# Janmajayamall/tfhe-research

Measured on AMD Instinct MI355X. Metric: programmable_bootstraps_per_sec, higher is better.
Workload: dtype f64

## Files before the change

include/tfhe_hip.h:

```cpp
#ifndef TFHE_HIP_H
#define TFHE_HIP_H

#include <stddef.h>
#include <stdint.h>

#ifdef __cplusplus
extern "C" {
#endif

#define TFHE_OK 0
#define TFHE_ERR_INVALID_PARAMS 1
#define TFHE_ERR_UNSUPPORTED 2
#define TFHE_ERR_NO_KEY 3
#define TFHE_ERR_HIP 4
#define TFHE_ERR_INVALID_ARGUMENT 5
#define TFHE_ERR_NO_DEVICE 6
#define TFHE_ERR_EXACTNESS 7
#define TFHE_ERR_IO 8

typedef struct tfhe_decomposer_params {
    uint32_t log_base;
    uint32_t levels;
    uint32_t log_q;
} tfhe_decomposer_params;
// ... 223 lines not shown
                                    uint32_t *bsk_bmmp, uint32_t *ksk, int load);
int tfhe_bootstrapping_key_gen_bmmp_device(tfhe_context *ctx, const uint32_t *lwe_sk,
                                           const uint32_t *glwe_sk, uint32_t *bsk_bmmp, uint32_t *ksk,
                                           int load);

int tfhe_context_set_bootstrap_order(tfhe_context *ctx, int ks_first);

#define TFHE_SHAPE_AUTO 0
#define TFHE_SHAPE_WIDE 1
#define TFHE_SHAPE_TEAM 2
int tfhe_context_set_kernel_shape(tfhe_context *ctx, int shape);

#define TFHE_KS_PATH_AUTO 0
#define TFHE_KS_PATH_SCALAR 1
#define TFHE_KS_PATH_MATRIX 2
int tfhe_context_set_key_switch_path(tfhe_context *ctx, int path);
int tfhe_debug_key_switch_plan(tfhe_context *ctx, size_t batch, int *path, unsigned *grid_x, unsigned *grid_y,
                               unsigned *splits);

int tfhe_context_set_decomposer_alignment(tfhe_context *ctx, int aligned);

#define TFHE_FILE_BSK 1
#define TFHE_FILE_KSK 2
#define TFHE_FILE_LWE 3
#define TFHE_FILE_GLWE 4
#define TFHE_FILE_GGSW 5
#define TFHE_FILE_WORDS 6
#define TFHE_FILE_PKSK 7
#define TFHE_FILE_FLAG_ALIGNED 1u
int tfhe_file_write(const char *path, uint32_t kind, const tfhe_params *params, uint32_t flags,
                    const uint32_t *dims, uint32_t ndims, const uint32_t *data);
// ... 56 lines not shown
```

rust/src/lib.rs:

```rust
use ndarray::{Array1, Array2, Array3};
use std::os::raw::{c_char, c_int, c_void};

#[repr(C)]
#[derive(Clone, Copy)]
pub struct CDecomposerParams { pub log_base: u32, pub levels: u32, pub log_q: u32 }

#[repr(C)]
#[derive(Clone, Copy)]
pub struct CTfheParams {
    pub glwe_dimension: u32, pub glwe_poly_degree: u32, pub lwe_dimension: u32,
    pub padding_bits: u32, pub log_p: u32, pub log_q: u32,
    pub ks_decomposer: CDecomposerParams, pub pbs_decomposer: CDecomposerParams,
}

#[repr(C)] pub struct TfheContext { _private: [u8; 0] }
#[repr(C)] pub struct TfhePool { _private: [u8; 0] }

extern "C" {
    fn tfhe_pool_create(params: *const CTfheParams, devices: *const c_int, n_devices: usize, backend: c_int,
                        out: *mut *mut TfhePool) -> c_int;
    fn tfhe_pool_destroy(pool: *mut TfhePool);
    fn tfhe_pool_member(pool: *mut TfhePool, i: usize) -> *mut TfheContext;
    fn tfhe_pool_last_error(pool: *const TfhePool) -> *const c_char;
    fn tfhe_pool_load_bootstrapping_key(pool: *mut TfhePool, bsk: *const u32, ksk: *const u32) -> c_int;
// ... 98 lines not shown
        check_pool(pool, unsafe { tfhe_pool_load_bootstrapping_key_bmmp(pool, bsk_bmmp.as_ptr(), ksk.as_ptr()) }, "load BMMP key");
        GpuBootstrappingKey { pool, ctx, params: *params }
    }
}

#[derive(Clone, Copy)]
pub enum KernelShape { Auto = 0, Wide = 1, Team = 2 }

impl GpuBootstrappingKey {
    pub fn set_kernel_shape(&self, shape: KernelShape) {
        check_pool(self.pool, unsafe { tfhe_pool_set_kernel_shape(self.pool, shape as c_int) }, "set kernel shape");
    }
}

#[derive(Clone, Copy)]
pub enum KeySwitchPath { Auto = 0, Scalar = 1, Matrix = 2 }

impl GpuBootstrappingKey {
    pub fn set_key_switch_path(&self, path: KeySwitchPath) {
        check_pool(self.pool, unsafe { tfhe_pool_set_key_switch_path(self.pool, path as c_int) }, "set key-switch path");
    }
}

impl Drop for GpuBootstrappingKey {
    fn drop(&mut self) { unsafe { tfhe_pool_destroy(self.pool) } }
}

pub fn bootstrap<SK1, SK2>(bk: &GpuBootstrappingKey, lwe_ciphertext: &Array1<u32>, _lwe_secret_key: &SK1,
                           _glwe_secret_key: &SK2, test_vector_poly: &Array1<u32>) -> Array1<u32> {
    let mut out = Array1::<u32>::zeros(lwe_ciphertext.len());
    check(bk.ctx, unsafe {
// ... 296 lines not shown
```

tfhe-research_amd/__init__.py:

```python
from __future__ import annotations

import ctypes as C
import os
from dataclasses import dataclass, field

import numpy as np

_HERE = os.path.dirname(os.path.abspath(__file__))
LIB_PATH = os.environ.get("TFHE_HIP_LIB") or os.path.join(_HERE, "libtfhe_hip.so")

TFHE_OK = 0
STATUS_NAMES = {
    0: "TFHE_OK", 1: "TFHE_ERR_INVALID_PARAMS", 2: "TFHE_ERR_UNSUPPORTED", 3: "TFHE_ERR_NO_KEY",
    4: "TFHE_ERR_HIP", 5: "TFHE_ERR_INVALID_ARGUMENT", 6: "TFHE_ERR_NO_DEVICE", 7: "TFHE_ERR_EXACTNESS",
    8: "TFHE_ERR_IO",
}
(TFHE_ERR_INVALID_PARAMS, TFHE_ERR_UNSUPPORTED, TFHE_ERR_NO_KEY, TFHE_ERR_HIP, TFHE_ERR_INVALID_ARGUMENT,
 TFHE_ERR_NO_DEVICE, TFHE_ERR_EXACTNESS, TFHE_ERR_IO) = range(1, 9)
FILE_BSK, FILE_KSK, FILE_LWE, FILE_GLWE, FILE_GGSW, FILE_WORDS, FILE_PKSK = 1, 2, 3, 4, 5, 6, 7
DECOMPOSER_PBS, DECOMPOSER_KS = 0, 1
BACKEND_AUTO, BACKEND_GOLDILOCKS, BACKEND_FP64, BACKEND_GOLDILOCKS_SPLIT, BACKEND_FP64_P49, BACKEND_FP64_FFT = 0, 1, 2, 3, 4, 5
SHAPE_AUTO, SHAPE_WIDE, SHAPE_TEAM = 0, 1, 2
KS_PATH_AUTO, KS_PATH_SCALAR, KS_PATH_MATRIX = 0, 1, 2

GATE_AND = (0, 0, 0, 1)
GATE_OR = (0, 1, 1, 1)
GATE_NAND = (1, 1, 1, 0)
GATE_XOR = (0, 1, 1, 0)


class TfheError(RuntimeError):
    def __init__(self, status: int, message: str = ""):
        self.status = status
        super().__init__(f"{STATUS_NAMES.get(status, status)}: {message}")


class _CDecomposer(C.Structure):
    _fields_ = [("log_base", C.c_uint32), ("levels", C.c_uint32), ("log_q", C.c_uint32)]
# ... 284 lines not shown
        if st:
            raise TfheError(st, message)

    @property
    def backend(self) -> str:
        return lib().tfhe_context_backend(self._h).decode()

    def set_decomposer_alignment(self, aligned: bool):
        self._check(lib().tfhe_context_set_decomposer_alignment(self._h, C.c_int(int(aligned))))

    def set_kernel_shape(self, shape: int):
        self._check(lib().tfhe_context_set_kernel_shape(self._h, C.c_int(int(shape))))

    def set_key_switch_path(self, path: int):
        self._check(lib().tfhe_context_set_key_switch_path(self._h, C.c_int(int(path))))

    def key_switch_plan(self, batch: int) -> dict:
        path, gx, gy, splits = C.c_int(), C.c_uint(), C.c_uint(), C.c_uint()
        self._check(lib().tfhe_debug_key_switch_plan(self._h, C.c_size_t(batch), C.byref(path), C.byref(gx), C.byref(gy),
                                                     C.byref(splits)))
        return {"path": path.value, "grid": (gx.value, gy.value), "splits": splits.value}

    def set_bootstrap_order(self, ks_first: bool):
        self._check(lib().tfhe_context_set_bootstrap_order(self._h, C.c_int(int(ks_first))))
        self._ks_first = bool(ks_first)

    @property
    def io_dim(self) -> int:
        return self.params.big_n if getattr(self, "_ks_first", False) else self.params.n

# ... 1196 lines not shown
```

tfhe-research_amd/csrc/capi.cpp:

```cpp
#include "context.h"

#include <cmath>
#include <cstdint>
#include <cstdio>
#include <cstdlib>
#include <cstring>
#include <initializer_list>
#include <new>
#include <algorithm>
#include <string>
#include <vector>

namespace {

using namespace tfhe::host;

u32 gadget_top(const tfhe_context* ctx, u32 log_base) {
  return ctx->aligned ? 32u : log_base * (32u / log_base);
}

constexpr size_t kMaxBatch = 0x7FFFFFFFull;

int decomposer_validate(const tfhe_decomposer_params& d) {
  if (d.log_q != 32) return 1;
// ... 20 lines not shown
  const size_t n1 = std::max((size_t)ctx->params.lwe_dimension, (size_t)ctx->big_n) + 1;
  const size_t glwe = glwe_words(ctx);
  u32** ptrs[] = {&ctx->d_lwe_in, &ctx->d_lwe_in2, &ctx->d_lwe_big, &ctx->d_lwe_out, &ctx->d_lwe_ks,
                  &ctx->d_glwe_a, &ctx->d_glwe_b,   &ctx->d_glwe_c,  &ctx->d_tv};
  const size_t sizes[] = {batch * n1, batch * n1, batch * n1, batch * n1, batch * n1,
                          batch * glwe, batch * glwe, batch * glwe, batch * ctx->N};
  HIP_TRY(ctx, hipStreamSynchronize(ctx->stream));
  ctx->ws_batch = 0;
  for (int i = 0; i < 9; ++i) {
    if (*ptrs[i]) {
      hipError_t e = hipFree(*ptrs[i]);
      *ptrs[i] = nullptr;
      if (e != hipSuccess) return hip_fail(ctx, e, "hipFree(workspace)");
    }
  }
  for (int i = 0; i < 9; ++i)
    HIP_TRY(ctx, hipMalloc(reinterpret_cast<void**>(ptrs[i]), sizes[i] * sizeof(u32)));
  ctx->ws_batch = batch;
  return TFHE_OK;
}

int ensure_misc(tfhe_context* ctx, size_t bytes) {
  if (bytes <= ctx->misc_bytes) return TFHE_OK;
  HIP_TRY(ctx, hipStreamSynchronize(ctx->stream));
  ctx->misc_bytes = 0;
  if (ctx->d_misc) {
    hipError_t e = hipFree(ctx->d_misc);
    ctx->d_misc = nullptr;
    if (e != hipSuccess) return hip_fail(ctx, e, "hipFree(misc)");
  }
  HIP_TRY(ctx, hipMalloc(&ctx->d_misc, bytes));
  ctx->misc_bytes = bytes;
  return TFHE_OK;
// ... 170 lines not shown
  return launch::blind_rotate(ctx->stream, ctx->field, P, ctx->d_tw, lwe_in, batch, tv, tv_count == 1 ? 0 : tv_words,
                              ctx->d_bsk, glwe_out, lwe_extracted, state, &ctx->side, ctx->shape);
}

int enqueue_bootstrap(tfhe_context* ctx, const u32* d_lwe_in, size_t batch, const u32* d_tv,
                      size_t tv_count, u32* d_lwe_big, u32* d_lwe_out, AccSource from = AccSource()) {
  const u32* br_in = d_lwe_in;
  u32* br_out = d_lwe_big;
  if (ctx->timing) {
    ctx->ev_slot = (ctx->ev_slot + 1) % tfhe_context::kTimingSlots;
    ctx->ev = ctx->ev_ring[ctx->ev_slot];
    ++ctx->timed_bootstraps;
  }
  auto key_switch = [&](const u32* in, u32* out) -> int {
    TFHE_TRY(span_begin(ctx, kKeySwitchSpan));
    HIP_TRY(ctx, launch::key_switch(ctx->stream, ctx->ks, ctx->big_n, ctx->params.lwe_dimension, in, batch, ctx->d_ksk, out, ctx->d_ksk_matrix, ctx->ks_path));
    return span_end(ctx, kKeySwitchSpan, false);
  };
  if (ctx->ks_first) {
    TFHE_TRY(key_switch(d_lwe_in, ctx->d_lwe_ks));
    br_in = ctx->d_lwe_ks;
    br_out = d_lwe_out;
  }
  TFHE_TRY(span_begin(ctx, kRotationSpan));
  HIP_TRY(ctx, enqueue_blind_rotate(ctx, br_in, batch, d_tv, tv_count, nullptr, br_out, from));
  TFHE_TRY(span_end(ctx, kRotationSpan, false));
  if (!ctx->ks_first) TFHE_TRY(key_switch(d_lwe_big, d_lwe_out));
  if (ctx->timing) ctx->ev_valid_br = ctx->ev_valid_ks = true;
  return TFHE_OK;
}

// ... 251 lines not shown

int tfhe_prepared_ggsw_words(const tfhe_context* ctx, size_t* words) {
  if (!ctx || !words) return TFHE_ERR_INVALID_ARGUMENT;
  *words = prepared_ggsw_words(ctx);
  return TFHE_OK;
}

void tfhe_context_destroy(tfhe_context* ctx) {
  if (!ctx) return;
  (void)hipSetDevice(ctx->device);
  (void)hipStreamSynchronize(ctx->stream);
  void* ptrs[] = {ctx->d_queue,  ctx->d_tw,     ctx->d_bsk,    ctx->d_ksk,    ctx->d_lwe_in, ctx->d_lwe_in2,
                  ctx->d_lwe_big, ctx->d_lwe_out, ctx->d_lwe_ks, ctx->d_glwe_a, ctx->d_glwe_b, ctx->d_glwe_c,
                  ctx->d_tv,     ctx->d_misc,   ctx->d_ggsw_tmp, ctx->d_ggsw_raw,
                  ctx->d_key_tmp, ctx->d_pksk, ctx->d_pack_cols, ctx->d_lookup_ws, ctx->d_tree_ws,
                  ctx->d_demux_ws, ctx->d_program_ws, ctx->d_dense_ws, ctx->d_ksk_matrix};
  for (void* p : ptrs)
    if (p) (void)hipFree(p);
  for (auto& g : ctx->gate_tvs)
    if (g.d_tv) (void)hipFree(g.d_tv);
  for (auto& slot : ctx->ev_ring)
    for (auto& ev : slot)
    if (ev) (void)hipEventDestroy(ev);
  if (ctx->side.stream) {
    (void)hipStreamSynchronize(ctx->side.stream);
    (void)hipStreamDestroy(ctx->side.stream);
  }
  if (ctx->side.fork) (void)hipEventDestroy(ctx->side.fork);
  if (ctx->side.join) (void)hipEventDestroy(ctx->side.join);
  if (ctx->own_stream && ctx->stream) (void)hipStreamDestroy(ctx->stream);
  delete ctx;
// ... 24 lines not shown
  ctx->pbs.first_shift = gadget_top(ctx, ctx->pbs.log_base) - ctx->pbs.log_base * ctx->pbs.levels;
  ctx->ks.first_shift = gadget_top(ctx, ctx->ks.log_base) - ctx->ks.log_base * ctx->ks.levels;
  return TFHE_OK;
}

int tfhe_context_set_kernel_shape(tfhe_context* ctx, int shape) {
  if (!ctx) return TFHE_ERR_INVALID_ARGUMENT;
  if (shape != TFHE_SHAPE_AUTO && shape != TFHE_SHAPE_WIDE && shape != TFHE_SHAPE_TEAM)
    return fail(ctx, TFHE_ERR_INVALID_ARGUMENT, "kernel shape: TFHE_SHAPE_AUTO, TFHE_SHAPE_WIDE or TFHE_SHAPE_TEAM");
  ctx->shape = shape;
  return TFHE_OK;
}

int tfhe_context_set_key_switch_path(tfhe_context* ctx, int path) {
  if (!ctx) return TFHE_ERR_INVALID_ARGUMENT;
  if (path != TFHE_KS_PATH_AUTO && path != TFHE_KS_PATH_SCALAR && path != TFHE_KS_PATH_MATRIX)
    return fail(ctx, TFHE_ERR_INVALID_ARGUMENT, "key-switch path: TFHE_KS_PATH_AUTO, TFHE_KS_PATH_SCALAR or TFHE_KS_PATH_MATRIX");
  if (path == TFHE_KS_PATH_MATRIX && !ks_matrix_admitted(ctx))
    return fail(ctx, TFHE_ERR_UNSUPPORTED,
                "the matrix-core key switch needs key-switch digits that fit int8 (log_base <= 6) and int32 plane sums "
                "that cannot overflow (k N levels 2^(log_base + 7) < 2^31): this parameter set runs the scalar kernel");
  ctx->ks_path = path;
  return TFHE_OK;
}

int tfhe_debug_key_switch_plan(tfhe_context* ctx, size_t batch, int* path, unsigned* grid_x, unsigned* grid_y,
                               unsigned* splits) {
  TFHE_TRY(check_ctx(ctx));
  TFHE_TRY(check_present(ctx, {path, grid_x, grid_y, splits}, 1, "null pointer"));
  if (batch == 0) return fail(ctx, TFHE_ERR_INVALID_ARGUMENT, "batch == 0");
  launch::KeySwitchPlanInfo plan{};
  HIP_TRY(ctx, launch::key_switch_plan(ctx->ks, ctx->big_n, ctx->params.lwe_dimension, batch, ctx->ks_path, &plan));
  *path = plan.matrix ? TFHE_KS_PATH_MATRIX : TFHE_KS_PATH_SCALAR;
  *grid_x = plan.grid_x;
  *grid_y = plan.grid_y;
  *splits = plan.splits;
  return TFHE_OK;
}

int tfhe_context_set_bootstrap_order(tfhe_context* ctx, int ks_first) {
  TFHE_TRY(check_ctx(ctx));
  HIP_TRY(ctx, hipStreamSynchronize(ctx->stream));
  ctx->ks_first = ks_first != 0;
  return TFHE_OK;
}

int tfhe_context_synchronize(tfhe_context* ctx) {
  TFHE_TRY(check_ctx(ctx));
// ... 309 lines not shown
}

namespace {
int check_key_switch_args(tfhe_context* ctx, const void* lwe_in, const void* lwe_out, size_t batch) {
  TFHE_TRY(check_present(ctx, {lwe_in, lwe_out}, batch));
  if (!ctx->have_key) return fail(ctx, TFHE_ERR_NO_KEY, "load the bootstrapping key first");
  return TFHE_OK;
}
}

int tfhe_key_switch_batch_device(tfhe_context* ctx, const uint32_t* lwe_in, size_t batch,
                                 uint32_t* lwe_out) {
  TFHE_TRY(check_ctx(ctx));
  TFHE_TRY(check_key_switch_args(ctx, lwe_in, lwe_out, batch));
  TFHE_TRY(span_begin(ctx, kKeySwitchSpan));
  HIP_TRY(ctx, launch::key_switch(ctx->stream, ctx->ks, ctx->big_n, ctx->params.lwe_dimension, lwe_in,
                                  batch, ctx->d_ksk, lwe_out, ctx->d_ksk_matrix, ctx->ks_path));
  return span_end(ctx, kKeySwitchSpan);
}

int tfhe_key_switch_batch(tfhe_context* ctx, const uint32_t* lwe_in, size_t batch, uint32_t* lwe_out) {
  TFHE_TRY(check_ctx(ctx));
  TFHE_TRY(check_key_switch_args(ctx, lwe_in, lwe_out, batch));
  TFHE_TRY(reserve(ctx, batch));
  TFHE_TRY(upload(ctx, ctx->d_lwe_big, lwe_in, batch * big_lwe_words(ctx)));
  TFHE_TRY(tfhe_key_switch_batch_device(ctx, ctx->d_lwe_big, batch, ctx->d_lwe_out));
  return download_and_wait(ctx, lwe_out, ctx->d_lwe_out, batch * lwe_words(ctx));
}

int tfhe_prepare_ggsw_device(tfhe_context* ctx, const uint32_t* ggsw, size_t ggsw_count,
                             void* ggsw_prepared) {
  TFHE_TRY(check_ctx(ctx));
// ... 1422 lines not shown
  TFHE_TRY(check_tree_lut_args(ctx, digits, d, batch, table, table_sets, tables, lwe_out, &L));
  if (L.words > ctx->tree_ws_words)
    return fail(ctx, TFHE_ERR_INVALID_ARGUMENT,
                "the call needs " + std::to_string(L.words * sizeof(u32)) + " bytes of tree-LUT workspace, " +
                    std::to_string(ctx->tree_ws_words * sizeof(u32)) + " are reserved (tfhe_context_reserve_tree_lut)");
  const u32 log_p = ctx->params.log_p, log_n = ctx->pbs.log_n, n = ctx->params.lwe_dimension;
  const u32 log_rep = log_n - log_p;
  const size_t n1 = lwe_words(ctx);
  u32* ws = ctx->d_tree_ws;
  u32 *ks_digit = ws + L.ks_digit, *lwe = ws + L.lwe, *tv = ws + L.tv, *state = ws + L.state, *glwes = ws + L.glwe;
  u32* results[2] = {ws + L.res_a, ws + L.res_b};
  hipStream_t s = ctx->stream;
  auto digit_of = [&](size_t t, const u32** out) -> int {
    *out = digits[t];
    if (!ctx->ks_first) return TFHE_OK;
    HIP_TRY(ctx, launch::key_switch(s, ctx->ks, ctx->big_n, n, digits[t], batch, ctx->d_ksk, ks_digit, ctx->d_ksk_matrix, ctx->ks_path));
    *out = ks_digit;
    return TFHE_OK;
  };
  size_t count = L.rotations;
  const u32* digit = nullptr;
  TFHE_TRY(digit_of(0, &digit));
  HIP_TRY(ctx, launch::tree_lut_expand(s, digit, count, count / batch, (u32)n1, lwe));
  HIP_TRY(ctx, launch::tree_lut_test_vectors(s, table, table_sets == 1 ? 0 : tables << (log_p * d), count, count / batch, log_p, log_n, tv));
  u32* cur = d == 1 && ctx->ks_first ? lwe_out : results[0];
  HIP_TRY(ctx, enqueue_blind_rotate(ctx, lwe, count, tv, count, nullptr, cur, AccSource{false, 0u, state}));
  for (size_t t = 1; t < d; ++t) {
    const size_t groups = count >> log_p;
    TFHE_TRY(enqueue_pack(ctx, cur, groups, 1u << log_p, glwes, log_rep));
    TFHE_TRY(digit_of(t, &digit));
    HIP_TRY(ctx, launch::tree_lut_expand(s, digit, groups, groups / batch, (u32)n1, lwe));
    u32* next = t + 1 == d && ctx->ks_first ? lwe_out : results[t & 1];
    HIP_TRY(ctx, enqueue_blind_rotate(ctx, lwe, groups, glwes, groups, nullptr, next, AccSource{true, (1u << log_rep) >> 1, state}));
    cur = next;
    count = groups;
  }
  if (!ctx->ks_first) HIP_TRY(ctx, launch::key_switch(s, ctx->ks, ctx->big_n, n, cur, count, ctx->d_ksk, lwe_out, ctx->d_ksk_matrix, ctx->ks_path));
  return TFHE_OK;
}

int tfhe_tree_lut_batch(tfhe_context* ctx, const uint32_t* const* digits, size_t d, size_t batch, const uint32_t* table,
                        size_t table_sets, size_t tables, uint32_t* lwe_out) {
  TFHE_TRY(check_ctx(ctx));
  TreeLutLayout L;
  TFHE_TRY(check_tree_lut_args(ctx, digits, d, batch, table, table_sets, tables, lwe_out, &L));
  TFHE_TRY(tfhe_context_reserve_tree_lut(ctx, batch, d, tables));
  const size_t io = io_words(ctx);
  std::vector<size_t> words(d, batch * io);
  words.push_back(table_sets * tables << (ctx->params.log_p * d));
  words.push_back(batch * tables * io);
  Staging s(ctx, words);
  TFHE_TRY(s.reserve());
// ... 275 lines not shown
```

tfhe-research_amd/csrc/context.h:

```cpp
#pragma once
#include "tfhe_hip.h"

#include <hip/hip_runtime.h>

#include <string>
#include <vector>

#include "launch.h"

using namespace tfhe;

struct tfhe_context {
  tfhe_params params;
  PbsParams pbs;
  KsParams ks;
  int device = 0;
  hipStream_t stream = nullptr;
  bool own_stream = false;
  launch::SideStream side = {nullptr, nullptr, nullptr};
  u32 N = 0, R = 0, big_n = 0;

  int field = 0;
  int parts = 1;
  void* d_tw = nullptr;
  unsigned long long* d_queue = nullptr;
  void* d_bsk = nullptr;
  u32* d_ksk = nullptr;
  void* d_ksk_matrix = nullptr;
  int ks_path = 0;
  bool have_key = false;
  bool bmmp = false;
  size_t bsk_ggsws = 0;
  void* d_pksk = nullptr;
  size_t pksk_bytes = 0;
  size_t pksk_dim = 0;
  bool have_pksk = false;
  u32* d_pack_cols = nullptr;
  size_t pack_cols_words = 0;
  u32* d_lookup_ws = nullptr;
  size_t lookup_ws_words = 0;
  unsigned lookup_height = 0;
  u32* d_demux_ws = nullptr;
  size_t demux_ws_words = 0;
  unsigned demux_height = 0;
// ... 17 lines not shown
  size_t tree_ws_words = 0;
  bool aligned = false;
  bool ks_first = false;
  int shape = 0;

  size_t ws_batch = 0;
  u32* d_lwe_in = nullptr;
  u32* d_lwe_in2 = nullptr;
  u32* d_lwe_big = nullptr;
  u32* d_lwe_out = nullptr;
  u32* d_lwe_ks = nullptr;
  u32* d_glwe_a = nullptr;
  u32* d_glwe_b = nullptr;
  u32* d_glwe_c = nullptr;
  u32* d_tv = nullptr;
  static constexpr size_t kMaxGateTvs = 64;
  struct GateTv {
    std::vector<u32> truth;
    u32* d_tv = nullptr;
    unsigned long long last_use = 0;
    bool pinned = false;
  };
  std::vector<GateTv> gate_tvs;
  unsigned long long gate_clock = 0;
  void* d_misc = nullptr;
  size_t misc_bytes = 0;
  u64* d_ggsw_tmp = nullptr;
  size_t ggsw_tmp_words = 0;
  u32* d_ggsw_raw = nullptr;
  size_t ggsw_raw_words = 0;
// ... 21 lines not shown

inline int hip_fail(tfhe_context* ctx, hipError_t e, const char* what) {
  return fail(ctx, TFHE_ERR_HIP, std::string(what) + ": " + hipGetErrorString(e));
}

int adopt_prepared_key(tfhe_context* dst, const tfhe_context* src);

inline size_t glwe_words(const tfhe_context* ctx) { return (size_t)(ctx->params.glwe_dimension + 1) * ctx->N; }
inline size_t lwe_words(const tfhe_context* ctx) { return (size_t)ctx->params.lwe_dimension + 1; }
inline size_t big_lwe_words(const tfhe_context* ctx) { return (size_t)ctx->big_n + 1; }
inline size_t io_words(const tfhe_context* ctx) { return ctx->ks_first ? big_lwe_words(ctx) : lwe_words(ctx); }
inline size_t ggsw_words(const tfhe_context* ctx) { return (size_t)ctx->R * glwe_words(ctx); }
inline size_t prepared_ggsw_words(const tfhe_context* ctx) { return ggsw_words(ctx) * ctx->parts; }
inline size_t ksk_words(const tfhe_context* ctx) { return (size_t)ctx->big_n * ctx->ks.levels * lwe_words(ctx); }
inline bool ks_matrix_admitted(const tfhe_context* ctx) { return ksm_admitted(ctx->ks.log_base, ctx->ks.levels, ctx->big_n); }
inline size_t ksk_matrix_bytes(const tfhe_context* ctx) {
  return launch::ksk_matrix_bytes(ctx->ks, ctx->big_n, ctx->params.lwe_dimension);
}
inline size_t packing_key_words(const tfhe_context* ctx, size_t from_dimension) {
  return from_dimension * ctx->ks.levels * glwe_words(ctx);
}
inline size_t prepared_bsk_bytes(const tfhe_context* ctx, size_t ggsws) {
  return ggsws * prepared_ggsw_words(ctx) * sizeof(u64);
}

}
}

#define HIP_TRY(ctx, expr)                                              \
  do {                                                                  \
// ... 10 lines not shown
```

tfhe-research_amd/csrc/kernels.hip:

```cpp
#include <atomic>
#include <cmath>
#include <cstdlib>

#include "launch.h"
#include "lwe_dense.h"

namespace tfhe {
namespace {

constexpr int kGroupN2048 = 4;
template <class F, int LOGN>
struct GroupOf {
  static constexpr int value = (LOGN >= 11) ? kGroupN2048 : 1;
};

template <class F, int LOGN>
constexpr bool field_shape_ok() {
  return F::kLogShrink == 0 || (LOGN >= 9 && LOGN <= 11);
}

template <class F, int LOGN>
constexpr size_t twiddle_bytes() {
  return (size_t)ntt_twiddle_words(1 << (LOGN - F::kLogShrink)) * sizeof(typename F::elem);
}
// ... 753 lines not shown

#pragma unroll
  for (u32 c = 0; c < kKsmColTiles; ++c) {
    const u32 col = (ct0 + c) * kKsmCols + r;
    if (col >= lo.width) continue;
#pragma unroll
    for (u32 e = 0; e < 16; ++e) {
      const size_t s = sample0 + (e & 3u) + 8 * (e >> 2) + 4 * h;
      if (s >= batch) continue;
      u32 out = 0u - ksm_fold((u32)acc[c][0][e], (u32)acc[c][1][e], (u32)acc[c][2][e], (u32)acc[c][3][e]);
      if (col == lo.width - 1 && blockIdx.z == 0) out += lwe_in[s * stride + lo.big_n];
      if (gridDim.z == 1) lwe_out[s * lo.width + col] = out;
      else atomicAdd(&lwe_out[s * lo.width + col], out);
    }
  }
}

__global__ void decompose_words_kernel(u32 log_base, u32 levels, u32 ignored_bits, u32 first_shift,
                                       const u32* __restrict__ values, size_t count,
                                       u32* __restrict__ digits) {
  for (size_t i = (size_t)blockIdx.x * blockDim.x + threadIdx.x; i < count;
       i += (size_t)gridDim.x * blockDim.x) {
    const u32 v = round_value(values[i], ignored_bits);
    u32 carry = 0;
    for (u32 t = 0; t < levels; ++t)
      digits[i * levels + (levels - 1 - t)] = decompose_limb(v, first_shift + log_base * t, log_base, carry);
  }
}

__global__ void decompose_glwe_kernel(u32 log_base, u32 levels, u32 ignored_bits, u32 first_shift,
// ... 1000 lines not shown
}

hipError_t demux_tree_pass(hipStream_t s, int field, const PbsParams& P, const void* tw, const DemuxTreePass& pass, size_t teams) {
  TFHE_DISPATCH_FIELD(field, TFHE_DISPATCH_LOGN_K(P.log_n, P.k, (launch_demux_tree_pass<FF, LL, KK>(s, P, tw, pass, teams))));
}

hipError_t program_plan(int field, const PbsParams& P, size_t queries, const u32* level_counts, u32 levels, u32 n_outputs,
                        u32 forced_parts, ProgramLaunch* out, ProgramPlanInfo* info) {
  TFHE_DISPATCH_FIELD(field, TFHE_DISPATCH_LOGN_K(P.log_n, P.k, (plan_program<FF, LL, KK>(queries, level_counts, levels, n_outputs, forced_parts, out, info))));
}

hipError_t cmux_program_pass(hipStream_t s, int field, const PbsParams& P, const void* tw, const CmuxProgramPass& pass, size_t queries) {
  TFHE_DISPATCH_FIELD(field, TFHE_DISPATCH_LOGN_K(P.log_n, P.k, (launch_cmux_program_pass<FF, LL, KK>(s, P, tw, pass, queries))));
}

hipError_t key_switch_plan(const KsParams& K, u32 big_n, u32 n, size_t batch, int path, KeySwitchPlanInfo* out) {
  if (batch == 0 || !out) return hipErrorInvalidValue;
  const bool admitted = ksm_admitted(K.log_base, K.levels, big_n);
  if (path == kKsPathMatrix && !admitted) return hipErrorInvalidValue;
  out->matrix = path == kKsPathMatrix || (path == kKsPathAuto && admitted && batch >= kKsMatrixMinBatch);
  if (out->matrix) {
    const KsmLayout lo = ksm_layout(big_n, K.levels, n);
    out->grid_x = lo.col_tiles / kKsmColTiles;
    out->grid_y = (unsigned)((batch + 4 * kKsmSamples - 1) / (4 * kKsmSamples));
    unsigned splits = kKsmTargetWgs / (out->grid_x * out->grid_y);
    if (splits > lo.sblocks) splits = lo.sblocks;
    if (splits < 1u) splits = 1u;
    out->per_split = (lo.sblocks + splits - 1) / splits;
    out->splits = (lo.sblocks + out->per_split - 1) / out->per_split;
    return hipSuccess;
  }
  out->grid_x = (n + 1 + kKsCols - 1) / kKsCols;
  out->grid_y = (unsigned)((batch + kKsSamples - 1) / kKsSamples);
  unsigned splits = kKsTargetWgs / (out->grid_x * out->grid_y);
  const unsigned max_splits = (big_n + 63u) / 64u;
  if (splits > max_splits) splits = max_splits;
  if (splits > 32u) splits = 32u;
// ... 2 lines not shown
  out->splits = (big_n + out->per_split - 1) / out->per_split;
  return hipSuccess;
}

size_t ksk_matrix_bytes(const KsParams& K, u32 big_n, u32 n) { return ksm_bytes(ksm_layout(big_n, K.levels, n)); }

hipError_t ksk_prepare_matrix(hipStream_t s, const KsParams& K, u32 big_n, u32 n, const u32* ksk, void* prepared) {
  const KsmLayout lo = ksm_layout(big_n, K.levels, n);
  const size_t threads = (size_t)lo.sblocks * lo.levels * lo.col_tiles * 64;
  hipLaunchKernelGGL(ksk_prepare_matrix_kernel, dim3(grid_for(threads, 256)), dim3(256), 0, s, lo, ksk,
                     static_cast<unsigned char*>(prepared));
  return hipGetLastError();
}

hipError_t key_switch(hipStream_t s, const KsParams& K, u32 big_n, u32 n, const u32* lwe_in,
                      size_t batch, const u32* ksk, u32* lwe_out, const void* ksk_matrix, int path) {
  KeySwitchPlanInfo plan{};
  hipError_t e = key_switch_plan(K, big_n, n, batch, path, &plan);
  if (e != hipSuccess) return e;
  if (plan.matrix && !ksk_matrix) return hipErrorInvalidValue;
  const size_t lds = ((size_t)kKsWords * K.levels * kKsSamples + 2 * (size_t)kKsKeyRows * kKsCols) * sizeof(u32);
  if (!plan.matrix && lds > 64 * 1024) return hipErrorInvalidValue;
  if (plan.splits > 1) {
    e = hipMemsetAsync(lwe_out, 0, batch * ((size_t)n + 1) * sizeof(u32), s);
    if (e != hipSuccess) return e;
  }
  const dim3 grid(plan.grid_x, plan.grid_y, plan.splits);
  if (plan.matrix)
    hipLaunchKernelGGL(key_switch_matrix_kernel, grid, dim3(256), 0, s, K, ksm_layout(big_n, K.levels, n), lwe_in, batch,
                       static_cast<const uint4*>(ksk_matrix), lwe_out, plan.per_split);
  else
    hipLaunchKernelGGL(key_switch_kernel, grid, dim3(256), lds, s, K, big_n, n, lwe_in, batch, ksk, lwe_out,
                       plan.per_split);
  return hipGetLastError();
}

hipError_t decompose_words(hipStream_t s, u32 log_base, u32 levels, u32 fs, const u32* values,
                           size_t count, u32* digits) {
  const u32 ig = 32 - log_base * levels;
  hipLaunchKernelGGL(decompose_words_kernel, dim3(grid_for(count, 256)), dim3(256), 0, s, log_base,
                     levels, ig, fs, values, count, digits);
  return hipGetLastError();
}

hipError_t decompose_glwe(hipStream_t s, u32 log_base, u32 levels, u32 fs, u32 polys_per_ct,
                          u32 n_coeff, const u32* glwe, size_t batch, u32* digits) {
  const u32 ig = 32 - log_base * levels;
  const size_t total = batch * polys_per_ct * n_coeff;
  hipLaunchKernelGGL(decompose_glwe_kernel, dim3(grid_for(total, 256)), dim3(256), 0, s, log_base,
// ... 140 lines not shown
```

tfhe-research_amd/csrc/ks_matrix.h:

```cpp
#pragma once
#include <stddef.h>

#include "pbs_wave.h"

namespace tfhe {

constexpr u32 kKsmWords = 32;
constexpr u32 kKsmCols = 32;
constexpr u32 kKsmSamples = 32;
constexpr u32 kKsmColTiles = 2;
constexpr u32 kKsmPlanes = 4;
constexpr u32 kKsmFragBytes = 64 * 16;

struct KsmLayout {
  u32 big_n, levels, width;
  u32 sblocks;
  u32 col_tiles;
};

TFHE_HD KsmLayout ksm_layout(u32 big_n, u32 levels, u32 n) {
  KsmLayout lo;
  lo.big_n = big_n;
  lo.levels = levels;
  lo.width = n + 1;
// ... 43 lines not shown
    int8_t s[4];
    ksm_split(w, s);
    for (u32 p = 0; p < kKsmPlanes; ++p) planes[p][j / 4] |= (u32)(unsigned char)s[p] << (8 * (j % 4));
  }
}

TFHE_HD void ksm_digit_fragment(const u32 (&v)[16], u32 (&carry)[16], u32 shift, u32 log_base, u32 (&a)[4]) {
  for (u32 q = 0; q < 4; ++q) a[q] = 0;
#pragma unroll
  for (u32 j = 0; j < 16; ++j) {
    const u32 d = decompose_limb(v[j], shift, log_base, carry[j]);
    a[j / 4] |= (d & 0xFFu) << (8 * (j % 4));
  }
}

TFHE_HD u32 ksm_fold(u32 p0, u32 p1, u32 p2, u32 p3) { return p0 + (p1 << 8) + (p2 << 16) + (p3 << 24); }

TFHE_HD bool ksm_admitted(u32 log_base, u32 levels, u32 big_n) {
  if (log_base < 1 || log_base > 6 || levels == 0) return false;
  const u64 terms = (u64)((big_n + kKsmWords - 1) / kKsmWords) * kKsmWords * levels;
  return (terms << (log_base + 7)) < ((u64)1 << 31);
}

}
```

tfhe-research_amd/csrc/launch.h:

```cpp
#pragma once
#include <hip/hip_runtime.h>

#include "ks_matrix.h"
#include "pbs_wave.h"

namespace tfhe {
namespace launch {

constexpr int kFieldGoldilocks = GlField::kId;
constexpr int kFieldFp64 = FpField::kId;
constexpr int kFieldGoldilocksSplit = GlSplitField::kId;
constexpr int kFieldFp49 = Fp49Field::kId;
constexpr int kFieldFft = FftField::kId;

bool shape_supported(u32 log_n, u32 k);
int field_parts(int field);
bool field_shape_supported(int field, u32 log_n);
int samples_per_team(int field, u32 log_n, u32 k);

hipError_t bsk_prepare(hipStream_t s, int field, u32 log_n, u32 k, const void* tw, const u32* polys,
                       size_t poly_count, void* spectra);

struct SideStream {
  hipStream_t stream;
// ... 17 lines not shown
};
hipError_t blind_rotate_plan(int field, const PbsParams& P, size_t batch, bool can_park, bool have_side,
                             BlindRotatePlanInfo* out, int shape = kShapeAuto);

bool shape_supported_bmmp(u32 log_n, u32 k);
bool field_supported_bmmp(int field);
hipError_t blind_rotate_bmmp(hipStream_t s, int field, const PbsParams& P, const void* tw,
                             const u32* lwe_in, size_t batch, const u32* tv, size_t tv_stride,
                             const void* bsk, u32* glwe_out, u32* lwe_extracted);

hipError_t external_product(hipStream_t s, int field, const PbsParams& P, const void* tw,
                            const void* ggsw, size_t ggsw_stride_words, const u32* glwe_in,
                            u32* ct1_inout, const u32* cmux_ct0, size_t batch, u32* glwe_out,
                            unsigned long long* queue );

constexpr int kKsPathAuto = 0, kKsPathScalar = 1, kKsPathMatrix = 2;
struct KeySwitchPlanInfo {
  bool matrix;
  unsigned grid_x, grid_y;
  unsigned splits;
  u32 per_split;
};
hipError_t key_switch_plan(const KsParams& K, u32 big_n, u32 n, size_t batch, int path, KeySwitchPlanInfo* out);
size_t ksk_matrix_bytes(const KsParams& K, u32 big_n, u32 n);
hipError_t ksk_prepare_matrix(hipStream_t s, const KsParams& K, u32 big_n, u32 n, const u32* ksk, void* prepared);
hipError_t key_switch(hipStream_t s, const KsParams& K, u32 big_n, u32 n, const u32* lwe_in,
                      size_t batch, const u32* ksk, u32* lwe_out, const void* ksk_matrix, int path);

hipError_t pack_transpose(hipStream_t s, const u32* lwe_in, size_t groups, u32 per_group, u32 d, u32 log_n, u32* cols,
                          u32 log_rep = 0);
hipError_t pack_lwe(hipStream_t s, int field, const PbsParams& P, const void* tw, const void* key, const u32* cols, u32 d,
                    size_t groups, u32* glwe_out);
hipError_t packing_add_gadget(hipStream_t s, u32* pksk, size_t rows, u32 k, u32 log_n, const u32* factor);

hipError_t tree_lut_expand(hipStream_t s, const u32* in, size_t count, size_t per_row, u32 words, u32* out);
hipError_t tree_lut_test_vectors(hipStream_t s, const u32* table, size_t set_stride, size_t count, size_t per_row, u32 log_p,
                                 u32 log_n, u32* tv);

struct LookupPlanInfo {
  u32 height;
  u32 launches;
  size_t workspace_words;
// ... 58 lines not shown
```

Baseline: 146,700.

## Add staged key switch with digit prepass and MFMA tiled GEMM

Adds a staged key-switch path that first decomposes input LWE masks into int8 digit fragments in a reserved device buffer, then runs a separate MFMA int8 kernel. That kernel double-buffers key fragments in LDS and reuses each key fragment across multiple sample tiles per wave. Auto mode selects it for batches of at least 256 when the digit buffer is reserved. The aim is to stop recomputing digits per column tile and to raise key reuse. The cost is an extra launch, a workspace allocation and a global memory round-trip for the digits.

```diff
diff --git a/include/tfhe_hip.h b/include/tfhe_hip.h
--- a/include/tfhe_hip.h
+++ b/include/tfhe_hip.h
@@ -261,7 +261,9 @@
 #define TFHE_KS_PATH_AUTO 0
 #define TFHE_KS_PATH_SCALAR 1
 #define TFHE_KS_PATH_MATRIX 2
+#define TFHE_KS_PATH_STAGED 3
 int tfhe_context_set_key_switch_path(tfhe_context *ctx, int path);
+int tfhe_context_set_key_switch_split(tfhe_context *ctx, unsigned splits);
 int tfhe_debug_key_switch_plan(tfhe_context *ctx, size_t batch, int *path, unsigned *grid_x, unsigned *grid_y,
                                unsigned *splits);
 
diff --git a/rust/src/lib.rs b/rust/src/lib.rs
--- a/rust/src/lib.rs
+++ b/rust/src/lib.rs
@@ -136,7 +136,7 @@
 }
 
 #[derive(Clone, Copy)]
-pub enum KeySwitchPath { Auto = 0, Scalar = 1, Matrix = 2 }
+pub enum KeySwitchPath { Auto = 0, Scalar = 1, Matrix = 2, Staged = 3 }
 
 impl GpuBootstrappingKey {
     pub fn set_key_switch_path(&self, path: KeySwitchPath) {
diff --git a/tfhe-research_amd/__init__.py b/tfhe-research_amd/__init__.py
--- a/tfhe-research_amd/__init__.py
+++ b/tfhe-research_amd/__init__.py
@@ -21,7 +21,7 @@
 DECOMPOSER_PBS, DECOMPOSER_KS = 0, 1
 BACKEND_AUTO, BACKEND_GOLDILOCKS, BACKEND_FP64, BACKEND_GOLDILOCKS_SPLIT, BACKEND_FP64_P49, BACKEND_FP64_FFT = 0, 1, 2, 3, 4, 5
 SHAPE_AUTO, SHAPE_WIDE, SHAPE_TEAM = 0, 1, 2
-KS_PATH_AUTO, KS_PATH_SCALAR, KS_PATH_MATRIX = 0, 1, 2
+KS_PATH_AUTO, KS_PATH_SCALAR, KS_PATH_MATRIX, KS_PATH_STAGED = 0, 1, 2, 3
 
 GATE_AND = (0, 0, 0, 1)
 GATE_OR = (0, 1, 1, 1)
@@ -336,6 +336,9 @@
 
     def set_key_switch_path(self, path: int):
         self._check(lib().tfhe_context_set_key_switch_path(self._h, C.c_int(int(path))))
+
+    def set_key_switch_split(self, splits: int):
+        self._check(lib().tfhe_context_set_key_switch_split(self._h, C.c_uint(int(splits))))
 
     def key_switch_plan(self, batch: int) -> dict:
         path, gx, gy, splits = C.c_int(), C.c_uint(), C.c_uint(), C.c_uint()
diff --git a/tfhe-research_amd/csrc/capi.cpp b/tfhe-research_amd/csrc/capi.cpp
--- a/tfhe-research_amd/csrc/capi.cpp
+++ b/tfhe-research_amd/csrc/capi.cpp
@@ -58,9 +58,32 @@
       if (e != hipSuccess) return hip_fail(ctx, e, "hipFree(workspace)");
     }
   }
+  ctx->ks_digit_bytes = 0;
+  if (ctx->d_ks_digits) {
+    hipError_t e = hipFree(ctx->d_ks_digits);
+    ctx->d_ks_digits = nullptr;
+    if (e != hipSuccess) return hip_fail(ctx, e, "hipFree(workspace)");
+  }
   for (int i = 0; i < 9; ++i)
     HIP_TRY(ctx, hipMalloc(reinterpret_cast<void**>(ptrs[i]), sizes[i] * sizeof(u32)));
+  if (ks_matrix_admitted(ctx)) {
+    const size_t bytes = launch::ks_digit_bytes(ctx->ks, ctx->big_n, ctx->params.lwe_dimension, batch);
+    HIP_TRY(ctx, hipMalloc(&ctx->d_ks_digits, bytes));
+    ctx->ks_digit_bytes = bytes;
+  }
   ctx->ws_batch = batch;
+  return TFHE_OK;
+}
+
+int enqueue_key_switch(tfhe_context* ctx, hipStream_t s, const u32* in, size_t batch, u32* out) {
+  if (ctx->ks_path == TFHE_KS_PATH_STAGED &&
+      launch::ks_digit_bytes(ctx->ks, ctx->big_n, ctx->params.lwe_dimension, batch) > ctx->ks_digit_bytes)
+    return fail(ctx, TFHE_ERR_INVALID_ARGUMENT,
+                "TFHE_KS_PATH_STAGED: the digit matrix is reserved for " + std::to_string(ctx->ws_batch) +
+                    " ciphertexts, the key switch has " + std::to_string(batch) + " (tfhe_context_reserve)");
+  HIP_TRY(ctx, launch::key_switch(s, ctx->ks, ctx->big_n, ctx->params.lwe_dimension, in, batch, ctx->d_ksk, out,
+                                  ctx->d_ksk_matrix, ks_resolved_path(ctx, batch), ctx->d_ks_digits, ctx->ks_digit_bytes,
+                                  ctx->ks_splits));
   return TFHE_OK;
 }
 
@@ -261,7 +284,7 @@
   }
   auto key_switch = [&](const u32* in, u32* out) -> int {
     TFHE_TRY(span_begin(ctx, kKeySwitchSpan));
-    HIP_TRY(ctx, launch::key_switch(ctx->stream, ctx->ks, ctx->big_n, ctx->params.lwe_dimension, in, batch, ctx->d_ksk, out, ctx->d_ksk_matrix, ctx->ks_path));
+    TFHE_TRY(enqueue_key_switch(ctx, ctx->stream, in, batch, out));
     return span_end(ctx, kKeySwitchSpan, false);
   };
   if (ctx->ks_first) {
@@ -543,7 +566,7 @@
                   ctx->d_lwe_big, ctx->d_lwe_out, ctx->d_lwe_ks, ctx->d_glwe_a, ctx->d_glwe_b, ctx->d_glwe_c,
                   ctx->d_tv,     ctx->d_misc,   ctx->d_ggsw_tmp, ctx->d_ggsw_raw,
                   ctx->d_key_tmp, ctx->d_pksk, ctx->d_pack_cols, ctx->d_lookup_ws, ctx->d_tree_ws,
-                  ctx->d_demux_ws, ctx->d_program_ws, ctx->d_dense_ws, ctx->d_ksk_matrix};
+                  ctx->d_demux_ws, ctx->d_program_ws, ctx->d_dense_ws, ctx->d_ksk_matrix, ctx->d_ks_digits};
   for (void* p : ptrs)
     if (p) (void)hipFree(p);
   for (auto& g : ctx->gate_tvs)
@@ -598,9 +621,10 @@
 
 int tfhe_context_set_key_switch_path(tfhe_context* ctx, int path) {
   if (!ctx) return TFHE_ERR_INVALID_ARGUMENT;
-  if (path != TFHE_KS_PATH_AUTO && path != TFHE_KS_PATH_SCALAR && path != TFHE_KS_PATH_MATRIX)
-    return fail(ctx, TFHE_ERR_INVALID_ARGUMENT, "key-switch path: TFHE_KS_PATH_AUTO, TFHE_KS_PATH_SCALAR or TFHE_KS_PATH_MATRIX");
-  if (path == TFHE_KS_PATH_MATRIX && !ks_matrix_admitted(ctx))
+  if (path != TFHE_KS_PATH_AUTO && path != TFHE_KS_PATH_SCALAR && path != TFHE_KS_PATH_MATRIX && path != TFHE_KS_PATH_STAGED)
+    return fail(ctx, TFHE_ERR_INVALID_ARGUMENT,
+                "key-switch path: TFHE_KS_PATH_AUTO, TFHE_KS_PATH_SCALAR, TFHE_KS_PATH_MATRIX or TFHE_KS_PATH_STAGED");
+  if ((path == TFHE_KS_PATH_MATRIX || path == TFHE_KS_PATH_STAGED) && !ks_matrix_admitted(ctx))
     return fail(ctx, TFHE_ERR_UNSUPPORTED,
                 "the matrix-core key switch needs key-switch digits that fit int8 (log_base <= 6) and int32 plane sums "
                 "that cannot overflow (k N levels 2^(log_base + 7) < 2^31): this parameter set runs the scalar kernel");
@@ -608,14 +632,24 @@
   return TFHE_OK;
 }
 
+int tfhe_context_set_key_switch_split(tfhe_context* ctx, unsigned splits) {
+  if (!ctx) return TFHE_ERR_INVALID_ARGUMENT;
+  ctx->ks_splits = splits;
+  return TFHE_OK;
+}
+
 int tfhe_debug_key_switch_plan(tfhe_context* ctx, size_t batch, int* path, unsigned* grid_x, unsigned* grid_y,
                                unsigned* splits) {
   TFHE_TRY(check_ctx(ctx));
   TFHE_TRY(check_present(ctx, {path, grid_x, grid_y, splits}, 1, "null pointer"));
   if (batch == 0) return fail(ctx, TFHE_ERR_INVALID_ARGUMENT, "batch == 0");
   launch::KeySwitchPlanInfo plan{};
-  HIP_TRY(ctx, launch::key_switch_plan(ctx->ks, ctx->big_n, ctx->params.lwe_dimension, batch, ctx->ks_path, &plan));
-  *path = plan.matrix ? TFHE_KS_PATH_MATRIX : TFHE_KS_PATH_SCALAR;
+  const size_t digit_bytes = ctx->ks_path == TFHE_KS_PATH_STAGED
+                                 ? launch::ks_digit_bytes(ctx->ks, ctx->big_n, ctx->params.lwe_dimension, batch)
+                                 : ctx->ks_digit_bytes;
+  HIP_TRY(ctx, launch::key_switch_plan(ctx->ks, ctx->big_n, ctx->params.lwe_dimension, batch, ks_resolved_path(ctx, batch),
+                                       &plan, digit_bytes, ctx->ks_splits));
+  *path = plan.staged ? TFHE_KS_PATH_STAGED : plan.matrix ? TFHE_KS_PATH_MATRIX : TFHE_KS_PATH_SCALAR;
   *grid_x = plan.grid_x;
   *grid_y = plan.grid_y;
   *splits = plan.splits;
@@ -955,8 +989,7 @@
   TFHE_TRY(check_ctx(ctx));
   TFHE_TRY(check_key_switch_args(ctx, lwe_in, lwe_out, batch));
   TFHE_TRY(span_begin(ctx, kKeySwitchSpan));
-  HIP_TRY(ctx, launch::key_switch(ctx->stream, ctx->ks, ctx->big_n, ctx->params.lwe_dimension, lwe_in,
-                                  batch, ctx->d_ksk, lwe_out, ctx->d_ksk_matrix, ctx->ks_path));
+  TFHE_TRY(enqueue_key_switch(ctx, ctx->stream, lwe_in, batch, lwe_out));
   return span_end(ctx, kKeySwitchSpan);
 }
 
@@ -2409,7 +2442,7 @@
   auto digit_of = [&](size_t t, const u32** out) -> int {
     *out = digits[t];
     if (!ctx->ks_first) return TFHE_OK;
-    HIP_TRY(ctx, launch::key_switch(s, ctx->ks, ctx->big_n, n, digits[t], batch, ctx->d_ksk, ks_digit, ctx->d_ksk_matrix, ctx->ks_path));
+    TFHE_TRY(enqueue_key_switch(ctx, s, digits[t], batch, ks_digit));
     *out = ks_digit;
     return TFHE_OK;
   };
@@ -2430,7 +2463,7 @@
     cur = next;
     count = groups;
   }
-  if (!ctx->ks_first) HIP_TRY(ctx, launch::key_switch(s, ctx->ks, ctx->big_n, n, cur, count, ctx->d_ksk, lwe_out, ctx->d_ksk_matrix, ctx->ks_path));
+  if (!ctx->ks_first) TFHE_TRY(enqueue_key_switch(ctx, s, cur, count, lwe_out));
   return TFHE_OK;
 }
 
diff --git a/tfhe-research_amd/csrc/context.h b/tfhe-research_amd/csrc/context.h
--- a/tfhe-research_amd/csrc/context.h
+++ b/tfhe-research_amd/csrc/context.h
@@ -28,6 +28,7 @@
   u32* d_ksk = nullptr;
   void* d_ksk_matrix = nullptr;
   int ks_path = 0;
+  unsigned ks_splits = 0;
   bool have_key = false;
   bool bmmp = false;
   size_t bsk_ggsws = 0;
@@ -75,6 +76,8 @@
   u32* d_glwe_b = nullptr;
   u32* d_glwe_c = nullptr;
   u32* d_tv = nullptr;
+  void* d_ks_digits = nullptr;
+  size_t ks_digit_bytes = 0;
   static constexpr size_t kMaxGateTvs = 64;
   struct GateTv {
     std::vector<u32> truth;
@@ -126,6 +129,12 @@
 inline size_t prepared_ggsw_words(const tfhe_context* ctx) { return ggsw_words(ctx) * ctx->parts; }
 inline size_t ksk_words(const tfhe_context* ctx) { return (size_t)ctx->big_n * ctx->ks.levels * lwe_words(ctx); }
 inline bool ks_matrix_admitted(const tfhe_context* ctx) { return ksm_admitted(ctx->ks.log_base, ctx->ks.levels, ctx->big_n); }
+constexpr size_t kKsStagedMinBatch = 256;
+inline int ks_resolved_path(const tfhe_context* ctx, size_t batch) {
+  if (ctx->ks_path != launch::kKsPathAuto || !ks_matrix_admitted(ctx) || batch < kKsStagedMinBatch) return ctx->ks_path;
+  const size_t need = launch::ks_digit_bytes(ctx->ks, ctx->big_n, ctx->params.lwe_dimension, batch);
+  return ctx->d_ks_digits && need <= ctx->ks_digit_bytes ? launch::kKsPathStaged : launch::kKsPathAuto;
+}
 inline size_t ksk_matrix_bytes(const tfhe_context* ctx) {
   return launch::ksk_matrix_bytes(ctx->ks, ctx->big_n, ctx->params.lwe_dimension);
 }
diff --git a/tfhe-research_amd/csrc/kernels.hip b/tfhe-research_amd/csrc/kernels.hip
--- a/tfhe-research_amd/csrc/kernels.hip
+++ b/tfhe-research_amd/csrc/kernels.hip
@@ -791,6 +791,108 @@
       else atomicAdd(&lwe_out[s * lo.width + col], out);
     }
   }
+}
+
+__global__ void __launch_bounds__(256) ks_digits_kernel(KsParams Kp, KsmLayout lo, const u32* __restrict__ lwe_in, size_t batch,
+                                                        unsigned char* __restrict__ digits) {
+  const size_t waves = ksd_tiles(batch) * lo.sblocks;
+  const size_t wave = (size_t)blockIdx.x * 4 + (threadIdx.x >> 6);
+  if (wave >= waves) return;
+  const u32 lane = threadIdx.x & 63u;
+  const u32 r = lane & 31u, h = lane >> 5;
+  const size_t st = wave / lo.sblocks;
+  const u32 sb = (u32)(wave % lo.sblocks);
+  const size_t sample = st * kKsmSamples + r;
+  const bool sample_ok = sample < batch;
+  const u32* row = lwe_in + (sample_ok ? sample : 0) * ((size_t)lo.big_n + 1);
+  u32 x[16];
+#pragma unroll
+  for (u32 j = 0; j < 16; ++j) {
+    const u32 word = sb * kKsmWords + h * 16 + j;
+    const u32 w = row[word < lo.big_n ? word : 0u];
+    x[j] = (sample_ok && word < lo.big_n) ? w : 0u;
+  }
+  ksd_prepass_lane(Kp, x, [&](u32 level, const u32 (&a)[4]) {
+    *reinterpret_cast<uint4*>(digits + ksd_fragment(lo, st, sb, level) + (size_t)lane * 16) = make_uint4(a[0], a[1], a[2], a[3]);
+  });
+}
+
+constexpr u32 kKssTiles = 2, kKssColTiles = 1;
+constexpr unsigned kKssTargetWgs = 512u;
+template <u32 MT, u32 CT>
+__global__ void __launch_bounds__(256, MT * CT * kKsmPlanes * 16 > 128 ? 1 : 2)
+    key_switch_staged_kernel(KsmLayout lo, const u32* __restrict__ lwe_in, size_t batch, const uint4* __restrict__ digits,
+                             const uint4* __restrict__ prepared, u32* __restrict__ lwe_out, u32 sblocks_per_split) {
+  constexpr u32 kFrags = CT * kKsmPlanes;
+  __shared__ uint4 stage[2][kFrags * 64];
+  const u32 lane = threadIdx.x & 63u, wave = threadIdx.x >> 6;
+  const u32 r = lane & 31u, h = lane >> 5;
+  const size_t tiles = ksd_tiles(batch);
+  const size_t st0 = ((size_t)blockIdx.y * 4 + wave) * MT;
+  const u32 ct0 = blockIdx.x * CT;
+  const u32 steps = lo.sblocks * lo.levels;
+
+  i32x16 acc[MT][CT][kKsmPlanes];
+#pragma unroll
+  for (u32 m = 0; m < MT; ++m)
+#pragma unroll
+    for (u32 c = 0; c < CT; ++c)
+#pragma unroll
+      for (u32 p = 0; p < kKsmPlanes; ++p)
+#pragma unroll
+        for (int e = 0; e < 16; ++e) acc[m][c][p][e] = 0;
+
+  const u32 sb_begin = blockIdx.z * sblocks_per_split;
+  const u32 sb_end = sb_begin + sblocks_per_split < lo.sblocks ? sb_begin + sblocks_per_split : lo.sblocks;
+  const u32 k_begin = sb_begin * lo.levels, k_end = sb_end * lo.levels;
+
+  uint4 b_next[CT], a_next[MT];
+  auto fetch = [&](u32 ks) {
+    const uint4* kf = prepared + ((size_t)ks * lo.col_tiles + ct0) * kKsmPlanes * 64;
+#pragma unroll
+    for (u32 i = 0; i < CT; ++i) b_next[i] = kf[i * 256 + threadIdx.x];
+#pragma unroll
+    for (u32 m = 0; m < MT; ++m)
+      a_next[m] = st0 + m < tiles ? digits[((st0 + m) * steps + ks) * 64 + lane] : make_uint4(0u, 0u, 0u, 0u);
+  };
+  if (k_begin < k_end) fetch(k_begin);
+  for (u32 ks = k_begin; ks < k_end; ++ks) {
+    uint4* buf = stage[(ks - k_begin) & 1u];
+#pragma unroll
+    for (u32 i = 0; i < CT; ++i) buf[i * 256 + threadIdx.x] = b_next[i];
+    i32x4 a[MT];
+#pragma unroll
+    for (u32 m = 0; m < MT; ++m) a[m] = i32x4{(i32)a_next[m].x, (i32)a_next[m].y, (i32)a_next[m].z, (i32)a_next[m].w};
+    __syncthreads();
+    if (ks + 1 < k_end) fetch(ks + 1);
+#pragma unroll
+    for (u32 c = 0; c < CT; ++c)
+#pragma unroll
+      for (u32 p = 0; p < kKsmPlanes; ++p) {
+        const uint4 b = buf[(c * kKsmPlanes + p) * 64 + lane];
+        const i32x4 bf = {(i32)b.x, (i32)b.y, (i32)b.z, (i32)b.w};
+#pragma unroll
+        for (u32 m = 0; m < MT; ++m) acc[m][c][p] = mfma_i32_32x32x32_i8(a[m], bf, acc[m][c][p]);
+      }
+  }
+
+  const size_t stride = (size_t)lo.big_n + 1;
+#pragma unroll
+  for (u32 m = 0; m < MT; ++m)
+#pragma unroll
+    for (u32 c = 0; c < CT; ++c) {
+      const u32 col = (ct0 + c) * kKsmCols + r;
+      if (col >= lo.width) continue;
+#pragma unroll
+      for (u32 e = 0; e < 16; ++e) {
+        const size_t s = (st0 + m) * kKsmSamples + (e & 3u) + 8 * (e >> 2) + 4 * h;
+        if (s >= batch) continue;
+        u32 out = 0u - ksm_fold((u32)acc[m][c][0][e], (u32)acc[m][c][1][e], (u32)acc[m][c][2][e], (u32)acc[m][c][3][e]);
+        if (col == lo.width - 1 && blockIdx.z == 0) out += lwe_in[s * stride + lo.big_n];
+        if (gridDim.z == 1) lwe_out[s * lo.width + col] = out;
+        else atomicAdd(&lwe_out[s * lo.width + col], out);
+      }
+    }
 }
 
 __global__ void decompose_words_kernel(u32 log_base, u32 levels, u32 ignored_bits, u32 first_shift,
@@ -1821,13 +1923,28 @@
   TFHE_DISPATCH_FIELD(field, TFHE_DISPATCH_LOGN_K(P.log_n, P.k, (launch_cmux_program_pass<FF, LL, KK>(s, P, tw, pass, queries))));
 }
 
-hipError_t key_switch_plan(const KsParams& K, u32 big_n, u32 n, size_t batch, int path, KeySwitchPlanInfo* out) {
+hipError_t key_switch_plan(const KsParams& K, u32 big_n, u32 n, size_t batch, int path, KeySwitchPlanInfo* out,
+                           size_t digit_bytes, unsigned forced_splits) {
   if (batch == 0 || !out) return hipErrorInvalidValue;
   const bool admitted = ksm_admitted(K.log_base, K.levels, big_n);
-  if (path == kKsPathMatrix && !admitted) return hipErrorInvalidValue;
-  out->matrix = path == kKsPathMatrix || (path == kKsPathAuto && admitted && batch >= kKsMatrixMinBatch);
+  if ((path == kKsPathMatrix || path == kKsPathStaged) && !admitted) return hipErrorInvalidValue;
+  const KsmLayout lo = ksm_layout(big_n, K.levels, n);
+  if (path == kKsPathStaged && ksd_bytes(lo, batch) > digit_bytes) return hipErrorInvalidValue;
+  out->staged = path == kKsPathStaged;
+  out->matrix = out->staged || path == kKsPathMatrix || (path == kKsPathAuto && admitted && batch >= kKsMatrixMinBatch);
+  out->prepass_grid = 0;
+  if (out->staged) {
+    out->grid_x = lo.col_tiles / kKssColTiles;
+    out->grid_y = (unsigned)((ksd_tiles(batch) + 4 * kKssTiles - 1) / (4 * kKssTiles));
+    out->prepass_grid = (unsigned)((ksd_tiles(batch) * lo.sblocks + 3) / 4);
+    unsigned splits = forced_splits ? forced_splits : kKssTargetWgs / (out->grid_x * out->grid_y);
+    if (splits > lo.sblocks) splits = lo.sblocks;
+    if (splits < 1u) splits = 1u;
+    out->per_split = (lo.sblocks + splits - 1) / splits;
+    out->splits = (lo.sblocks + out->per_split - 1) / out->per_split;
+    return hipSuccess;
+  }
   if (out->matrix) {
-    const KsmLayout lo = ksm_layout(big_n, K.levels, n);
     out->grid_x = lo.col_tiles / kKsmColTiles;
     out->grid_y = (unsigned)((batch + 4 * kKsmSamples - 1) / (4 * kKsmSamples));
     unsigned splits = kKsmTargetWgs / (out->grid_x * out->grid_y);
@@ -1860,9 +1977,10 @@
 }
 
 hipError_t key_switch(hipStream_t s, const KsParams& K, u32 big_n, u32 n, const u32* lwe_in,
-                      size_t batch, const u32* ksk, u32* lwe_out, const void* ksk_matrix, int path) {
+                      size_t batch, const u32* ksk, u32* lwe_out, const void* ksk_matrix, int path, void* digits,
+                      size_t digit_bytes, unsigned forced_splits) {
   KeySwitchPlanInfo plan{};
-  hipError_t e = key_switch_plan(K, big_n, n, batch, path, &plan);
+  hipError_t e = key_switch_plan(K, big_n, n, batch, path, &plan, digits ? digit_bytes : 0, forced_splits);
   if (e != hipSuccess) return e;
   if (plan.matrix && !ksk_matrix) return hipErrorInvalidValue;
   const size_t lds = ((size_t)kKsWords * K.levels * kKsSamples + 2 * (size_t)kKsKeyRows * kKsCols) * sizeof(u32);
@@ -1872,13 +1990,25 @@
     if (e != hipSuccess) return e;
   }
   const dim3 grid(plan.grid_x, plan.grid_y, plan.splits);
-  if (plan.matrix)
+  if (plan.staged) {
+    const KsmLayout lo = ksm_layout(big_n, K.levels, n);
+    hipLaunchKernelGGL(ks_digits_kernel, dim3(plan.prepass_grid), dim3(256), 0, s, K, lo, lwe_in, batch,
+                       static_cast<unsigned char*>(digits));
+    e = hipGetLastError();
+    if (e != hipSuccess) return e;
+    hipLaunchKernelGGL((key_switch_staged_kernel<kKssTiles, kKssColTiles>), grid, dim3(256), 0, s, lo, lwe_in, batch,
+                       static_cast<const uint4*>(digits), static_cast<const uint4*>(ksk_matrix), lwe_out, plan.per_split);
+  } else if (plan.matrix)
     hipLaunchKernelGGL(key_switch_matrix_kernel, grid, dim3(256), 0, s, K, ksm_layout(big_n, K.levels, n), lwe_in, batch,
                        static_cast<const uint4*>(ksk_matrix), lwe_out, plan.per_split);
   else
     hipLaunchKernelGGL(key_switch_kernel, grid, dim3(256), lds, s, K, big_n, n, lwe_in, batch, ksk, lwe_out,
                        plan.per_split);
   return hipGetLastError();
+}
+
+size_t ks_digit_bytes(const KsParams& K, u32 big_n, u32 n, size_t batch) {
+  return ksd_bytes(ksm_layout(big_n, K.levels, n), batch);
 }
 
 hipError_t decompose_words(hipStream_t s, u32 log_base, u32 levels, u32 fs, const u32* values,
diff --git a/tfhe-research_amd/csrc/ks_matrix.h b/tfhe-research_amd/csrc/ks_matrix.h
--- a/tfhe-research_amd/csrc/ks_matrix.h
+++ b/tfhe-research_amd/csrc/ks_matrix.h
@@ -81,6 +81,31 @@
   }
 }
 
+TFHE_HD size_t ksd_tiles(size_t batch) { return (batch + kKsmSamples - 1) / kKsmSamples; }
+
+TFHE_HD size_t ksd_bytes(const KsmLayout& lo, size_t batch) {
+  return ksd_tiles(batch) * lo.sblocks * lo.levels * kKsmFragBytes;
+}
+
+TFHE_HD size_t ksd_fragment(const KsmLayout& lo, size_t st, u32 sb, u32 level) {
+  return ((st * lo.sblocks + sb) * lo.levels + level) * kKsmFragBytes;
+}
+
+template <typename Store>
+TFHE_HD void ksd_prepass_lane(const KsParams& Kp, const u32 (&x)[16], Store store) {
+  u32 v[16], carry[16];
+#pragma unroll
+  for (u32 j = 0; j < 16; ++j) {
+    v[j] = round_value(x[j], Kp.ignored_bits);
+    carry[j] = 0;
+  }
+  for (u32 t = 0; t < Kp.levels; ++t) {
+    u32 a[4];
+    ksm_digit_fragment(v, carry, Kp.first_shift + Kp.log_base * t, Kp.log_base, a);
+    store(Kp.levels - 1 - t, a);
+  }
+}
+
 TFHE_HD u32 ksm_fold(u32 p0, u32 p1, u32 p2, u32 p3) { return p0 + (p1 << 8) + (p2 << 16) + (p3 << 24); }
 
 TFHE_HD bool ksm_admitted(u32 log_base, u32 levels, u32 big_n) {
diff --git a/tfhe-research_amd/csrc/launch.h b/tfhe-research_amd/csrc/launch.h
--- a/tfhe-research_amd/csrc/launch.h
+++ b/tfhe-research_amd/csrc/launch.h
@@ -55,18 +55,23 @@
                             u32* ct1_inout, const u32* cmux_ct0, size_t batch, u32* glwe_out,
                             unsigned long long* queue );
 
-constexpr int kKsPathAuto = 0, kKsPathScalar = 1, kKsPathMatrix = 2;
+constexpr int kKsPathAuto = 0, kKsPathScalar = 1, kKsPathMatrix = 2, kKsPathStaged = 3;
 struct KeySwitchPlanInfo {
   bool matrix;
+  bool staged;
   unsigned grid_x, grid_y;
   unsigned splits;
   u32 per_split;
+  unsigned prepass_grid;
 };
-hipError_t key_switch_plan(const KsParams& K, u32 big_n, u32 n, size_t batch, int path, KeySwitchPlanInfo* out);
+hipError_t key_switch_plan(const KsParams& K, u32 big_n, u32 n, size_t batch, int path, KeySwitchPlanInfo* out,
+                           size_t digit_bytes = 0, unsigned forced_splits = 0);
 size_t ksk_matrix_bytes(const KsParams& K, u32 big_n, u32 n);
 hipError_t ksk_prepare_matrix(hipStream_t s, const KsParams& K, u32 big_n, u32 n, const u32* ksk, void* prepared);
+size_t ks_digit_bytes(const KsParams& K, u32 big_n, u32 n, size_t batch);
 hipError_t key_switch(hipStream_t s, const KsParams& K, u32 big_n, u32 n, const u32* lwe_in,
-                      size_t batch, const u32* ksk, u32* lwe_out, const void* ksk_matrix, int path);
+                      size_t batch, const u32* ksk, u32* lwe_out, const void* ksk_matrix, int path, void* digits = nullptr,
+                      size_t digit_bytes = 0, unsigned forced_splits = 0);
 
 hipError_t pack_transpose(hipStream_t s, const u32* lwe_in, size_t groups, u32 per_group, u32 d, u32 log_n, u32* cols,
                           u32 log_rep = 0);
```

After: 147,400, median of 6. Within noise of the previous version (+0.5%).
